# markrosoft/se-195-project-ray-tracer

Hardware: AMD Instinct MI355X
Metric: Mrays/sec + ms/frame @1920x1080 Cornell-64spp, 1/2/4/8 GPU; % HBM roofline (higher is better)
Workload: dtype f32; 1 GPU; smallpt Cornell 1920x1080 64spp RadiancePathTracing, one frame per step; spp=64, spheres=9, rows_per_gpu=1080, parallelism=single GPU

## Files before the change

se-195-project-ray-tracer_amd/csrc/smallpt.hip:

```cpp
#include "rt_common.h"
#include "rt_glibc_math.h"
#include "spt_policy.h"
#include "spt_layout.h"
#include "spt_accept.h"
#include "spt_rng.h"

namespace rt {
namespace smallpt {

using namespace sptlayout;
namespace acc = sptaccept;
constexpr float EPS = acc::EPS;
constexpr float PI_F = 3.14159265358979323846f;
constexpr int DIFF = 0, SPEC = 1;
#ifndef RT_SPT_QUNROLL
#define RT_SPT_QUNROLL 3
#endif

struct SphereGeo { float4 g; };

__device__ __forceinline__ float get_random_f(uint32_t &s0, uint32_t &s1)
{
    return __uint_as_float(sptrng::draw<true>(s0, s1));
}
// ... 55 lines not shown
    return id;
}

constexpr float DET_SAFE = 0x1p-96f;
template <class G, class F, class T>
__device__ __forceinline__ bool for_spheres_bf(const G &geo, const ray3 &r, F &&accept, T &&trip)
{
    const auto roots = [&](int i, float &t1, float &t2) {
        const float4 g = geo.at(i);
        const float opx = g.x - r.o.x, opy = g.y - r.o.y, opz = g.z - r.o.z;
        const float b = opx * r.d.x + opy * r.d.y + opz * r.d.z;
        const float det = b * b - (opx * opx + opy * opy + opz * opz) + g.w;
        const float sd = sqrt_nr(det);
        t1 = b - sd;
        t2 = b + sd;
        return fabsf(det);
    };
    bool bad = false;
    int i = geo.count() - 1;
#pragma unroll 1
    for (; i >= RT_SPT_QUNROLL - 1; i -= RT_SPT_QUNROLL) {
        float t1[RT_SPT_QUNROLL], t2[RT_SPT_QUNROLL];
        float m = roots(i, t1[0], t2[0]);
#pragma unroll
        for (int j = 1; j < RT_SPT_QUNROLL; j++) m = __builtin_fminf(m, roots(i - j, t1[j], t2[j]));
        trip(RT_SPT_QUNROLL);
#pragma unroll
        for (int j = 0; j < RT_SPT_QUNROLL; j++) accept(i - j, RT_SPT_QUNROLL - 1 - j, t1[j], t2[j]);
        bad = bad || m < DET_SAFE;
    }
#pragma unroll 1
    for (; i >= 0; i--) {
        float t1, t2;
        bad = bad || roots(i, t1, t2) < DET_SAFE;
        trip(1);
        accept(i, 0, t1, t2);
    }
    return bad;
}

template <bool COUNT, bool KEYED, class G>
__device__ __forceinline__ int query_bf(const G &geo, const ray3 &r, float &t, int &first)
{
    const float t_in = t;
    int id = -1;
    bool bad = false;
    if constexpr (KEYED && COUNT) {
        uint32_t tb = acc::limit_key(t_in);
        bad = for_spheres_bf(geo, r, [&](int i, int, float t1, float t2) {
            const bool take = acc::nearest_accept(tb, t1, t2);
            id = take ? i : id;
            first = (first < 0 && take) ? i : first;
        }, [](int) {});
        t = acc::nearest_result(tb, t_in);
    } else if constexpr (KEYED) {
        uint32_t tb = acc::limit_key(t_in);
        int since = -(1 << 30);
        bad = for_spheres_bf(geo, r, [&](int, int after, float t1, float t2) {
            since = acc::nearest_accept(tb, t1, t2) ? after : since;
        }, [&](int k) { since += k; });
        id = since;
        t = acc::nearest_result(tb, t_in);
    } else {
#pragma unroll RT_SPT_QUNROLL
        for (int i = geo.count() - 1; i >= 0; i--) {
            const float4 g = geo.at(i);
            const float opx = g.x - r.o.x, opy = g.y - r.o.y, opz = g.z - r.o.z;
            const float b = opx * r.d.x + opy * r.d.y + opz * r.d.z;
            const float det = b * b - (opx * opx + opy * opy + opz * opz) + g.w;
            bad = bad || fabsf(det) < DET_SAFE;
            const float sd = sqrt_nr(det);
            const float t1 = b - sd, t2 = b + sd;
            const float d = t1 > EPS ? t1 : t2;
            const bool take = d > EPS && d < t;
            t = take ? d : t;
            id = take ? i : id;
            if (COUNT) first = (first < 0 && take) ? i : first;
        }
    }
    if (wave_any(bad)) {
        t = t_in;
        first = -1;
        id = query<COUNT>(geo, r, t, first);
    }
    return id;
}

template <bool COUNT, class G>
__device__ __forceinline__ void query2_bf(const G &geo, const ray3 &r, float &t, int &id, const ray3 &rs, bool sh,
                                          float &ts, int &ids, int &firsts)
{
    const float t_in = t, ts_in = ts;
    int first = -1;
    id = -1;
    ids = -1;
    bool bad = false, occ = false;
#pragma unroll RT_SPT_QUNROLL
    for (int i = geo.count() - 1; i >= 0; i--) {
        const float4 g = geo.at(i);
        {
            const float opx = g.x - r.o.x, opy = g.y - r.o.y, opz = g.z - r.o.z;
            const float b = opx * r.d.x + opy * r.d.y + opz * r.d.z;
            const float det = b * b - (opx * opx + opy * opy + opz * opz) + g.w;
            bad = bad || fabsf(det) < 0x1p-96f;
            const float sd = sqrt_nr(det);
            const float t1 = b - sd, t2 = b + sd;
            const float d = t1 > EPS ? t1 : t2;
            const bool take = d > EPS && d < t;
            t = take ? d : t;
            id = take ? i : id;
        }
        {
            const float opx = g.x - rs.o.x, opy = g.y - rs.o.y, opz = g.z - rs.o.z;
            const float b = opx * rs.d.x + opy * rs.d.y + opz * rs.d.z;
            const float det = b * b - (opx * opx + opy * opy + opz * opz) + g.w;
            bad = bad || (sh && fabsf(det) < 0x1p-96f);
            const float sd = sqrt_nr(det);
            const float t1 = b - sd, t2 = b + sd;
            const float d = t1 > EPS ? t1 : t2;
            const bool take = d > EPS && d < ts;
            if (COUNT) {
                ts = take ? d : ts;
                ids = take ? i : ids;
                firsts = (firsts < 0 && take) ? i : firsts;
            } else {
                occ = occ || take;
            }
        }
    }
    if (!COUNT) ids = occ ? 0 : -1;
    if (wave_any(bad)) {
        t = t_in;
        id = query<COUNT>(geo, r, t, first);
        ts = ts_in;
        firsts = -1;
        ids = query<COUNT>(geo, rs, ts, firsts);
    }
}

template <class G>
__device__ __forceinline__ bool shadow_bf(const G &geo, const ray3 &rs, float maxt, bool have)
{
    uint32_t near = acc::KEY_NONE;
    const bool bad = for_spheres_bf(geo, rs, [&](int, int, float t1, float t2) { acc::any_accept(near, t1, t2); }, [](int) {});
    bool occ = acc::any_result(near, maxt);
    if (wave_any(have && bad)) {
        float ts = maxt;
        int first = -1;
        occ = query<false>(geo, rs, ts, first) >= 0;
    }
    return occ;
}

#include "spt_walk.h"

struct Counts { unsigned isect, isectp, samples; unsigned long long tests; };

#ifdef RT_SPT_PROF
enum { PB_ITER, PB_SHADOW, PB_NEAREST, PB_DIFF, PB_SPEC, PB_REFR, PB_LIGHT, PB_BOUNCE, PB_DONE,
       PB_WCALL, PB_WSTEP, PB_WLEAF, PB_WSHADE, PB_FLUSH,
       PB_FL_THRESH, PB_FL_SLOT, PB_FL_ENDS, PB_FL_EMIT, PB_FL_DRAIN, PB_N };
__device__ unsigned long long g_spt_prof[2 * PB_N];
#define SPT_PROF(b)                                                                        \
    do {                                                                                   \
        prof_l[b]++;                                                                       \
        if ((int)(threadIdx.x & 63) == __builtin_ctzll(__builtin_amdgcn_read_exec())) prof_w[b]++; \
    } while (0)
#else
#define SPT_PROF(b) do {} while (0)
#endif

#ifdef RT_SPT_TRACE
__device__ uint4 *g_spt_trace;
__device__ int g_spt_only_group = -1;
#endif

__device__ __forceinline__ int to_int(float x)
{
    const float c = (x < 0.f) ? 0.f : ((x > 1.f) ? 1.f : x);
    return rt::cvt_i32_x86(rtm::powf(c, 1.f / 2.2f) * 255.f + .5f);
}
__device__ __forceinline__ uint32_t pack_rgb(float r, float g, float b)
{
    return (uint32_t)to_int(r) | ((uint32_t)to_int(g) << 8) | ((uint32_t)to_int(b) << 16);
}

template <bool DL, bool COUNT, int GEO, bool DUAL = false, bool RAYS = false, int CG = 0>
__global__ void __launch_bounds__(1024, variant_of(GEO, DL, DUAL, COUNT, RAYS, CG).min_waves())
render_kernel(const rt_sphere *__restrict__ spheres, int nspheres, rt_camera cam,
              float *__restrict__ colors, const uint32_t *seeds_in,
              uint32_t *seeds_out, uint32_t *__restrict__ pixels, int w, int h,
              int row_begin, int row_end, int tiles_x, int ntiles, int nslots, int gstride, int first_sample,
              int nsamples, int prio_sched, const int *__restrict__ group_order, unsigned *__restrict__ group_cost,
              const float4 *__restrict__ g_geo, const float4 *__restrict__ g_emi,
              const float4 *__restrict__ g_col, const float4 *__restrict__ g_lrec, int nlights,
              BvhView bvh, unsigned long long *__restrict__ counters, int *__restrict__ work, int split,
              int nheavy, int sflags)
{
    constexpr Variant V = variant_of(GEO, DL, DUAL, COUNT, RAYS, CG);
    constexpr bool LDS = V.lds();
    constexpr bool PERSIST = V.persist();
    constexpr bool PARK = V.park();
    constexpr bool DQ = V.dq();
    constexpr int WAVE_DW = wave_dwords(DQ);
    constexpr int SQ_RING = RING_FIELD_DW;
    extern __shared__ __attribute__((aligned(16))) char smem[];
    const int park_off = park_offset(V, nspheres, nlights);
    constexpr bool HELD = V.held_addr();
    const auto park_ptr = [&]() {
        int t = (int)threadIdx.x;
        if constexpr (!HELD) asm volatile("" : "+v"(t));
        return (float *)(smem + park_off + PARK_HEAD_BYTES) + (t >> 6) * WAVE_DW + (t & 63);
    };
    const auto ring_ptr = [&]() {
        const int t = (int)threadIdx.x;
        return (float *)(smem + park_off + PARK_HEAD_BYTES) + (t >> 6) * WAVE_DW + RING_BASE_DW;
    };
    if (PARK && threadIdx.x == 0) {
        float4 *pc = (float4 *)(smem + park_off);
        pc[0] = make_float4(cam.x.x, cam.x.y, cam.x.z, 1.f / w);
        pc[1] = make_float4(cam.y.x, cam.y.y, cam.y.z, 1.f / h);
        pc[2] = make_float4(cam.dir.x, cam.dir.y, cam.dir.z, 0.f);
        pc[3] = make_float4(cam.orig.x, cam.orig.y, cam.orig.z, 0.f);
    }
    if (PARK && !LDS) __syncthreads();
    Scene S;
    if (LDS) {
        float4 *s = (float4 *)smem;
        const int nrec = scene_records(nspheres, nlights);
        for (int i = threadIdx.x; i < nrec; i += blockDim.x) s[i] = g_geo[i];
        __syncthreads();
        S.geo = s; S.emi = s + nspheres; S.col = s + 2 * nspheres; S.lrec = s + 3 * nspheres;
    } else {
        S.geo = g_geo; S.emi = g_emi; S.col = g_col; S.lrec = g_lrec;
    }
    S.nlights = nlights;
    S.n = nspheres;
    const DynGeo geo{S.geo, S.n};
    const uint4 *wL = (const uint4 *)smem;
    unsigned *wstk = nullptr;
    if (GEO == GEO_WIDE) {
        uint4 *d = (uint4 *)smem;
        for (int i = threadIdx.x; i < 7 * bvh.wnodes; i += blockDim.x) d[i] = bvh.wnode[i];
        if (COUNT)
            for (int i = threadIdx.x; i < 2 * bvh.wnodes; i += blockDim.x) d[7 * bvh.wnodes + i] = bvh.wmax[i];
        wstk = (unsigned *)(smem + wide_stack_offset(bvh.wnodes, COUNT)) +
               (size_t)(threadIdx.x >> 6) * WIDE_LEVEL_DW * (bvh.wdepth - 1);
        __syncthreads();
    }

    const int lane = threadIdx.x & 63, wave = threadIdx.x >> 6;
    constexpr bool SCHED = V.sched();
    constexpr bool CALLS = COUNT || RAYS;
    Counts cnt = {0, 0, 0, 0};
    SPT_PROF_ONLY(unsigned prof_l[PB_N] = {}, prof_w[PB_N] = {};)
    const int hs = PERSIST ? sptpolicy::split_hs(split) : 0;
    const int hw = sptpolicy::split_hw(split) ? sptpolicy::split_hw(split) : (4 << hs);
    const int nitems = 4 * nslots;
    const int n1 = PERSIST ? min(sptpolicy::nheavy_n1(nheavy), nitems) : 0;
    const int n2 = PERSIST ? min(sptpolicy::nheavy_n2(nheavy), nitems - n1) : 0;
    const int nwork = (n1 << hs) + (nitems - n1);
    const int nstatic = PERSIST ? min(min(hw, (int)(blockDim.x >> 6)) * (int)gridDim.x, n1 << hs) : 0;
    const auto fetch = [&]() {
        int v = 0;
        if (lane == __builtin_ctzll(__builtin_amdgcn_read_exec())) {
            v = -1;
            if (wave < hw && n1 > 0) {
                const int hv = atomicAdd(work + 2, 1) + nstatic;
                if (hv < (n1 << hs)) v = hv;
            }
            if (v < 0 && wave < 4 && n2 > 0) {
                const int hv = atomicAdd(work + 1, 1);
                if (hv < n2) v = (n1 << hs) + hv;
            }
            if (v < 0) v = (n1 << hs) + n2 + atomicAdd(work, 1);
        }
        return __builtin_amdgcn_readfirstlane(v);
    };
    int f = ((wave >> 2) * (int)gridDim.x + (int)blockIdx.x) * 4 + (wave & 3);
    if (PERSIST) {
        const int fs = wave * (int)gridDim.x + (int)blockIdx.x;
        f = (wave < hw && fs < (n1 << hs)) ? fs : __builtin_amdgcn_readfirstlane(fetch());
    }
    while (!PERSIST || f < nwork) {
    const bool heavy_ = f < (n1 << hs);
    const bool coop = GEO == GEO_WIDE && CG != 0 && heavy_;
    const int cg = coop ? CG : 0;
    const int item = heavy_ ? f >> hs : f - (n1 << hs) + n1;
    const int sub = heavy_ ? f & ((1 << hs) - 1) : 0;
    const int slot = item >> 2;
    const int grp = group_order ? (slot < nslots ? group_order[slot] : -1) : slot;
    const bool gvalid = (unsigned)grp < (unsigned)((ntiles + 3) >> 2);
    const int tile = grp * 4 + (item & 3);
    const int li = coop ? (sub << (6 - hs)) + (lane >> hs) : lane;
    const bool lead = !coop || (lane & (cg - 1)) == 0;
    unsigned long long t_start = 0;
    if (SCHED) t_start = __builtin_amdgcn_s_memrealtime();
    constexpr bool GSTORE = V.gstore();
#define GS_BASE() (smem + (size_t)((threadIdx.x >> 6) >> 2) * GS_BYTES)
    if (GSTORE) {
        if ((threadIdx.x & 255) == 0) *(int *)(GS_BASE() + GS_COUNT_OFF) = 0;
        __syncthreads();
    }
    int x = (tile % tiles_x) * 8 + (li & 7);
    int y = row_begin + (tile / tiles_x) * 8 * gstride + (li >> 3);
    const bool refill = COUNT && PERSIST && !heavy_;
    bool active = gvalid && tile < ntiles && x < w && y < row_end
                  SPT_TRACE(&& (g_spt_only_group < 0 || grp == g_spt_only_group));
    SPT_TRACE(unsigned tr_walk = 0, tr_leaf = 0, tr_trips = 0, tr_leafruns = 0, tr_queries = 0;
              const unsigned long long tr_c0 = __builtin_amdgcn_s_memtime();
              const unsigned long long tr_t0 = __builtin_amdgcn_s_memrealtime();
              unsigned tr_iters = 0;)
    if (active || refill || DQ) {
        int i = (h - y - 1) * w + x;
// ... 74 lines not shown
                        if (SCHED && group_cost) {
                            const unsigned dur = (unsigned)__builtin_amdgcn_s_memrealtime() - pix_t0;
                            if (sptpolicy::sflags_cost_max(sflags)) atomicMax(&group_cost[pgrp], dur);
                            else atomicAdd(&group_cost[pgrp], dur);
                        }
                    }
                    const unsigned long long need = __builtin_amdgcn_ballot_w64(want);
                    const int ncl = __builtin_popcountll(need);
                    const int rank = __builtin_amdgcn_mbcnt_hi((unsigned)(need >> 32),
                                                               __builtin_amdgcn_mbcnt_lo((unsigned)need, 0u));
                    const bool more = rf_p + ncl > 64;
                    const int f2 = more ? fetch() : nwork;
                    if (want) {
                        const int pos = rf_p + rank;
                        const int mf = pos < 64 ? rf_f : f2, mp = pos < 64 ? pos : pos - 64;
                        px_ok = false;
                        if (mf >= nwork) {
                            exhausted = true;
                        } else {
                            const int it = mf - (n1 << hs) + n1, sl = it >> 2;
                            const int g = group_order ? (sl < nslots ? group_order[sl] : -1) : sl;
                            const int tl = g * 4 + (it & 3);
                            x = (tl % tiles_x) * 8 + (mp & 7);
                            y = row_begin + (tl / tiles_x) * 8 * gstride + (mp >> 3);
                            if ((unsigned)g < (unsigned)((ntiles + 3) >> 2) && tl < ntiles && x < w && y < row_end) {
                                i = (h - y - 1) * w + x;
                                s0 = seeds_in[2 * (size_t)i];
                                s1 = seeds_in[2 * (size_t)i + 1];
                                col = mk(0.f, 0.f, 0.f);
                                if (first_sample > 0)
                                    col = mk(colors[3 * (size_t)i], colors[3 * (size_t)i + 1], colors[3 * (size_t)i + 2]);
                                k = 0;
                                need_cam = nsamples > 0;
                                px_ok = true;
                                pgrp = g;
                                pix_t0 = (unsigned)__builtin_amdgcn_s_memrealtime();
                            }
                        }
                    }
                    if (more) {
                        rf_f = f2;
                        rf_p += ncl - 64;
                    } else {
                        rf_p += ncl;
                    }
                }
            }
            if (need_bounce || need_cam) {
                SPT_PROF(PB_BOUNCE);
                const float f1 = get_random_f(s0, s1), f2 = get_random_f(s0, s1);
                const float x1 = __builtin_fmaf(f1, .5f, -1.f), x2 = __builtin_fmaf(f2, .5f, -1.f);
                const v3 wv = nl;
                const v3 a = (fabsf(wv.x) > .1f) ? mk(0.f, 1.f, 0.f) : mk(1.f, 0.f, 0.f);
                const v3 cu = vxcross(a, wv);
                float4 cmx = make_float4(cam.x.x, cam.x.y, cam.x.z, invW), cmy = make_float4(cam.y.x, cam.y.y, cam.y.z, invH);
                float4 cmd = make_float4(cam.dir.x, cam.dir.y, cam.dir.z, 0.f);
                float4 cmo = make_float4(cam.orig.x, cam.orig.y, cam.orig.z, 0.f);
                if constexpr (PARK) {
                    int o = park_off;
                    asm volatile("" : "+s"(o));
                    const float4 *pc = (const float4 *)(smem + o);
                    cmx = pc[0]; cmy = pc[1]; cmd = pc[2]; cmo = pc[3];
                }
                const float kcx = (x + __builtin_fmaf(f1, .5f, -1.5f)) * cmx.w - .5f;
                const float kcy = (y + __builtin_fmaf(f2, .5f, -1.5f)) * cmy.w - .5f;
                const v3 rdir = mk(cmx.x * kcx + cmy.x * kcy + cmd.x,
                                   cmx.y * kcx + cmy.y * kcy + cmd.y,
                                   cmx.z * kcx + cmy.z * kcy + cmd.z);
                const v3 vn = vnorm(need_bounce ? cu : rdir);
                if (need_bounce) {
                    const float r2s = sqrt_exact(x2);
                    const v3 v = vxcross(wv, vn);
                    float sn1, cs1, r2c;
                    if constexpr (V.draw_trig()) {
                        rtm::sincos_2pi_draw_bits(__float_as_uint(f1), x1, sn1, cs1);
                        r2c = sqrt_nr(1 - x2);
                    } else {
                        rtm::sincosf(2.f * PI_F * x1, sn1, cs1);
                        r2c = sqrt_exact(1 - x2);
                    }
                    const v3 u = vsmul(cs1 * r2s, vn);
                    v3 nd = vadd(u, vsmul(sn1 * r2s, v));
                    nd = vadd(nd, vsmul(r2c, wv));
                    ray.d = nd;
                } else {
                    v3 rorig = vsmul(0.1f, rdir);
                    rorig = vadd(rorig, mk(cmo.x, cmo.y, cmo.z));
                    ray.o = rorig;
                    ray.d = vn;
                }
                need_bounce = need_cam = false;
            }
            const bool live = !DQ || k < nsamples;
            bool drain = false;
            if constexpr (DQ) {
                drain = !wave_any(live);
                if (drain && q_count == 0) break;
            } else if (k >= nsamples) {
                if (!refill || exhausted) break;
                continue;
            }
            if (!refill && !wave_any(k < prio_next)) {
                prio_level++;
                prio_next = prio_level < 3 ? (nsamples * sptpolicy::prio_bound(prio_sched, prio_level)) >> 8 : nsamples;
                if (prio_level == 1) __builtin_amdgcn_s_setprio(2);
                else if (prio_level == 2) __builtin_amdgcn_s_setprio(1);
                else __builtin_amdgcn_s_setprio(0);
            }

            SPT_PROF(PB_ITER);
            SPT_TRACE(tr_iters++;)
            float t = (shadow && !DUAL) ? lmax : 1e20f;
            int first = -1;
            int id;
            bool done = false, lights = false, a_R = false;
            bool pushed = false;
            if constexpr (DQ) {
                id = -1;
                if (live) id = query_bf<COUNT, V.key_accept()>(geo, ray, t, first);
                bool f_emit = false, f_ends = false, f_diff = false;
                if (live && npend > 0) {
                    bool emit = false;
                    if (id >= 0) {
                        const float4 oe = S.emi[id];
                        emit = !((oe.x == 0.f) && (oe.x == 0.f) && (oe.z == 0.f));
                        f_diff = !emit && __float_as_int(oe.w) == DIFF;
                    }
                    f_emit = emit && specular;
                    f_ends = id < 0 || emit || depth >= 6;
                }
                while (true) {
                    const bool force = (f_emit && npend > npark) || (f_ends && npark > 0) || (f_diff && npend == 2);
                    if (q_count == 0 || !(sptpolicy::sq_flush(q_count, q_T) || drain || wave_any(force))) break;
                    const int m = sptpolicy::sq_pop(q_count);
                    const int e = sptpolicy::sq_wrap(q_head + lane);
                    const float *rg = ring_ptr();
                    ray3 rs;
                    rs.o = mk(rg[e], rg[SQ_RING + e], rg[2 * SQ_RING + e]);
                    rs.d = mk(rg[3 * SQ_RING + e], rg[4 * SQ_RING + e], rg[5 * SQ_RING + e]);
                    const float maxt = rg[6 * SQ_RING + e];
                    const bool have = lane < m;
                    SPT_PROF_ONLY(if (have) prof_l[PB_FLUSH]++; if (lane == 0) prof_w[PB_FLUSH]++;)
                    SPT_PROF_ONLY({
                        const int why = sptpolicy::sq_flush(q_count, q_T)        ? PB_FL_THRESH
                                        : wave_any(f_diff && npend == 2)         ? PB_FL_SLOT
                                        : wave_any(f_ends && npark > 0)          ? PB_FL_ENDS
                                        : wave_any(f_emit && npend > npark)      ? PB_FL_EMIT
                                                                                 : PB_FL_DRAIN;
                        _Pragma("unroll") for (int b = PB_FL_THRESH; b <= PB_FL_DRAIN; b++) {
                            if (have && b == why) prof_l[b]++;
                            if (lane == 0 && b == why) prof_w[b]++;
                        }
                    })
                    const bool occ = shadow_bf(geo, rs, maxt, have);
                    const unsigned long long unocc = __builtin_amdgcn_ballot_w64(have && !occ);
                    while (npend > 0) {
                        const int rel = sptpolicy::sq_rel(pidx & 255, q_head);
                        if (rel >= m) break;
                        const bool lit = (unocc >> rel) & 1ull;
                        if (npark > 0) {
                            float *p = park_ptr();
                            if (lit) {
                                p[64 * SLOT_RAD] = p[64 * SLOT_RAD] + pc0.x;
                                p[64 * (SLOT_RAD + 1)] = p[64 * (SLOT_RAD + 1)] + pc0.y;
                                p[64 * (SLOT_RAD + 2)] = p[64 * (SLOT_RAD + 2)] + pc0.z;
                            }
                            npark--;
                            if (npark == 0)
                                fold(mk(p[64 * SLOT_RAD], p[64 * (SLOT_RAD + 1)], p[64 * (SLOT_RAD + 2)]),
                                     first_sample + k - 1);
                        } else if (lit) {
                            rad = vadd(rad, pc0);
                        }
                        npend--;
                        pidx >>= 8;
                        if (npend > 0) {
                            const float *p = park_ptr();
                            pc0 = mk(p[64 * SLOT_PEND], p[64 * (SLOT_PEND + 1)], p[64 * (SLOT_PEND + 2)]);
                        }
                    }
                    q_head = __builtin_amdgcn_readfirstlane(sptpolicy::sq_wrap(q_head + m));
                    q_count = __builtin_amdgcn_readfirstlane(q_count - m);
                }
            } else if constexpr (DUAL) {
                if (wave_any(shadow)) {
                    float ts = lmax;
                    int ids, firsts = -1;
                    ray3 rs;
                    rs.o = hit;
                    rs.d = sdir;
                    query2_bf<COUNT>(geo, ray, t, id, rs, shadow, ts, ids, firsts);
                    if (shadow) {
                        SPT_PROF(PB_SHADOW);
                        cnt.isectp++;
                        cnt.tests += firsts >= 0 ? (unsigned)(S.n - firsts) : (unsigned)S.n;
                        if (ids < 0) {
                            const float4 le = S.lrec[2];
                            const v3 ld = vsmul(lw, mk(le.x, le.y, le.z));
                            rad = vadd(rad, vmul(thr, ld));
                        }
                        shadow = false;
                        done = fin;
                    }
                } else {
                    id = query_bf<COUNT, V.key_accept()>(geo, ray, t, first);
                }
            } else if constexpr (GEO == GEO_BVH) {
                SPT_TRACE(const unsigned long long tr_w0 = __builtin_amdgcn_s_memtime(); tr_queries += !walking;)
                if (!walking) bvh_begin<COUNT>(bvh, ray, shadow, t, walk);
                walking = !bvh_walk<COUNT>(bvh, ray, shadow, walk);
                SPT_TRACE(tr_walk += (unsigned)(__builtin_amdgcn_s_memtime() - tr_w0);)
                if (walking) continue;
                t = walk.t;
                id = walk.id;
                first = id;
            } else if constexpr (GEO == GEO_WIDE) {
                SPT_TRACE(const unsigned long long tr_w0 = __builtin_amdgcn_s_memtime(); tr_queries += !walking;)
                if (!walking) wide_begin<COUNT>(bvh, ray, shadow, t, walk);
                if constexpr (CG != 0)
                    walking = coop ? !wide_walk_coop<COUNT, (CG ? CG : 8)>(bvh, wL, wstk, ray, shadow, walk, split)
                                   : !wide_walk<COUNT>(bvh, wL, wstk, ray, shadow, walk, split);
                else
                    walking = !wide_walk<COUNT>(bvh, wL, wstk, ray, shadow, walk, split);
                SPT_TRACE(tr_walk += (unsigned)(__builtin_amdgcn_s_memtime() - tr_w0);)
                if (walking) continue;
                SPT_PROF(PB_WSHADE);
                t = walk.t;
                id = walk.id;
                first = id;
            } else {
                id = query_bf<COUNT, V.key_accept()>(geo, ray, t, first);
            }
            float dp = 0.f, inv_sign = 1.f;
            if (DQ && !live) {
            } else if (DUAL && fin) {
            } else if (shadow && !DUAL) {
                SPT_PROF(PB_SHADOW);
                cnt.isectp++;
                cnt.tests += first >= 0 ? (unsigned)(S.n - first) : (unsigned)S.n;
                if (id < 0) {
                    const float4 le = S.lrec[3 * li + 2];
                    lsum = vadd(lsum, vsmul(lw, mk(le.x, le.y, le.z)));
                }
                li++;
                lights = true;
                shadow = false;
            } else {
                cnt.isect++;
                cnt.tests += S.n;
                if (id < 0) {
                    done = true;
                } else {
                    SPT_PROF(PB_NEAREST);
                    const float4 og = S.geo[id], oe = S.emi[id], oc = S.col[id];
                    hit = vadd(ray.o, vsmul(t, ray.d));
                    v3 normal = vsub(hit, mk(og.x, og.y, og.z));
                    normal = vnorm(normal);
                    dp = vdot(normal, ray.d);
                    inv_sign = -1.f * (dp > 0 ? 1.f : -1.f);
                    nl = vsmul(inv_sign, normal);
                    const int refl = __float_as_int(oe.w);
                    if (!((oe.x == 0.f) && (oe.x == 0.f) && (oe.z == 0.f))) {
                        if (specular) {
                            v3 e = vsmul(fabsf(dp), mk(oe.x, oe.y, oe.z));
                            e = vmul(thr, e);
                            rad = vadd(rad, e);
                        }
                        done = true;
                    } else if (refl == DIFF) {
                        SPT_PROF(PB_DIFF);
                        specular = false;
                        thr = vmul(thr, mk(oc.x, oc.y, oc.z));
                        lsum = mk(0.f, 0.f, 0.f);
                        li = 0;
                        lights = true;
                    } else if (refl == SPEC) {
                        SPT_PROF(PB_SPEC);
                        specular = true;
                        v3 nd = vsmul(2.f * vdot(normal, ray.d), normal);
                        nd = vsub(ray.d, nd);
                        thr = vmul(thr, mk(oc.x, oc.y, oc.z));
                        ray.d = nd;
                    } else {
                        SPT_PROF(PB_REFR);
                        specular = true;
                        a_R = true;
                    }
                    depth++;
                    done = done || (!lights && !a_R && depth > 6);
                }
            }

            bool a_L = lights && li < S.nlights;
            bool lights_done = lights && !a_L;
            const bool was_R = a_R;
            const auto pass_a = [&](const bool with_r) {
                {
                    SPT_PROF(PB_LIGHT);
                    const int lj = li < S.nlights ? li : 0;
                    const float4 lg = S.lrec[3 * lj];
                    const float4 lc = S.lrec[3 * lj + 1];
                    const v3 normal = vsmul(inv_sign, nl);
                    const bool into = dp <= 0.f;
                    const float nnt = into ? nc / nt : nt / nc;
                    const float ddn = inv_sign * dp;
                    const float cos2t = 1.f - nnt * nnt * (1.f - ddn * ddn);
                    const bool tir = cos2t < 0.f;
                    float g1 = 2.f, x2 = 0.f;
                    if (a_L || (with_r && !tir)) g1 = get_random_f(s0, s1);
                    const float x1 = __builtin_fmaf(g1, .5f, -1.f);
                    if (a_L) x2 = get_random(s0, s1);
                    const float zz = 1.f - 2.f * x2;
                    const float q = 1.f - zz * zz;
                    const float sq = sqrt_exact((!with_r || a_L) ? ((0.f > q) ? 0.f : q) : (tir ? 1.f : cos2t));
                    float sp_sin, sp_cos;
                    if constexpr (V.draw_trig()) rtm::sincos_2pi_draw_bits(__float_as_uint(g1), x1, sp_sin, sp_cos);
                    else rtm::sincosf(2.f * PI_F * x1, sp_sin, sp_cos);
                    const v3 unit = mk(sq * sp_cos, sq * sp_sin, zz);
                    v3 sp = vsmul(lc.w, unit);
                    sp = vadd(sp, mk(lg.x, lg.y, lg.z));
                    const v3 vl = vsub(sp, hit);
                    const float kk = (into ? 1.f : -1.f) * (ddn * nnt + sq);
                    const v3 vr = vsub(vsmul(nnt, ray.d), vsmul(kk, normal));
                    const v3 vv = (!with_r || a_L) ? vl : vr;
                    const float dd = vdot(vv, vv);
                    float len, ilen;
                    if (!wave_any(!sqrt_nr_ok(dd))) {
                        len = sqrt_nr(dd);
                        ilen = rcp_nr(len);
                    } else {
                        len = sqrt_rn(dd);
                        ilen = 1.f / len;
                    }
                    const v3 vn = vsmul(ilen, vv);
                    const float dv = vdot(vn, (!with_r || a_L) ? unit : normal);
                    const float wo = -dv;
                    const float wi = vdot(vn, nl);
                    const bool lit = a_L && !(dv > 0.f) && wi > 0.f;
                    const float a = nt - nc, b = nt + nc;
                    const float R0 = a * a / (b * b);
                    const float c = 1 - (into ? -ddn : dv);
                    const float Re = R0 + (1 - R0) * c * c * c * c * c;
                    const float Tr = 1.f - Re;
                    const float P = .25f + .5f * Re;
                    const bool refl_pick = x1 < P;
                    const bool l_lane = !with_r || a_L;
                    const float num = l_lane ? (4.f * PI_F * lc.w * lc.w) * wi * wo : (refl_pick ? Re : Tr);
                    const float den = l_lane ? len * len : (refl_pick ? P : 1.f - P);
                    const float quo = num / den;
                    unsigned long long pm = 0;
                    if constexpr (DQ) pm = __builtin_amdgcn_ballot_w64(lit);
                    if (!with_r || a_L) {
                        if (DQ && lit) {
                            const int rank = __builtin_amdgcn_mbcnt_hi((unsigned)(pm >> 32),
                                                                       __builtin_amdgcn_mbcnt_lo((unsigned)pm, 0u));
                            const int pos = sptpolicy::sq_push_pos(q_head, q_count, rank);
                            float *rg = ring_ptr();
                            rg[pos] = hit.x;
                            rg[SQ_RING + pos] = hit.y;
                            rg[2 * SQ_RING + pos] = hit.z;
                            rg[3 * SQ_RING + pos] = vn.x;
                            rg[4 * SQ_RING + pos] = vn.y;
                            rg[5 * SQ_RING + pos] = vn.z;
                            rg[6 * SQ_RING + pos] = len - EPS;
                            const float4 le = S.lrec[2];
                            const v3 c = vmul(thr, vsmul(quo, mk(le.x, le.y, le.z)));
                            if (npend == 0) {
                                pc0 = c;
                                pidx = pos;
                            } else {
                                float *p = park_ptr();
                                p[64 * SLOT_PEND] = c.x;
                                p[64 * (SLOT_PEND + 1)] = c.y;
                                p[64 * (SLOT_PEND + 2)] = c.z;
                                pidx |= pos << 8;
                            }
                            npend++;
                            pushed = true;
                            a_L = false;
                            lights_done = true;
                        } else if (lit) {
                            if (DUAL) {
                                sdir = vn;
                            } else {
                                ray.d = vn;
                            }
                            lmax = len - EPS;
                            lw = quo;
                            shadow = true;
                            a_L = false;
                            if (DUAL) lights_done = true;
                        } else {
                            li++;
                            a_L = li < S.nlights;
                            lights_done = !a_L;
                        }
                    } else {
                        const float4 oc = S.col[id];
                        v3 nd = vsmul(2.f * dp, normal);
                        nd = vsub(ray.d, nd);
                        if (tir) {
                            thr = vmul(thr, mk(oc.x, oc.y, oc.z));
                            ray.d = nd;
                        } else {
                            thr = vsmul(quo, thr);
                            thr = vmul(thr, mk(oc.x, oc.y, oc.z));
                            ray.d = refl_pick ? nd : vn;
                        }
                        a_R = false;
                    }
                }
            };
            if ((GEO == GEO_BVH || GEO == GEO_WIDE) && sptpolicy::sflags_no_refr(sflags)) {
                if (a_L) pass_a(false);
            } else if (a_L || a_R) {
                pass_a(true);
            }
            if (S.nlights > 1) {
                while (wave_any(a_L)) {
                    if (a_L) pass_a(false);
                }
            }
            if constexpr (DQ)
                q_count = __builtin_amdgcn_readfirstlane(
                    q_count + __builtin_popcountll(__builtin_amdgcn_ballot_w64(pushed)));
            if (was_R) done = depth > 6;
            if (lights_done) {
                if (!DUAL) rad = vadd(rad, vmul(thr, lsum));
                if (DL) {
                    done = true;
                } else if (depth > 6) {
                    (void)get_random(s0, s1);
                    (void)get_random(s0, s1);
                    if (DUAL && shadow) fin = true;
                    else done = true;
                } else {
                    need_bounce = true;
                }
            }
            if (done) {
                SPT_PROF(PB_DONE);
                const int current = first_sample + k;
                if constexpr (DQ) {
                    if (npend > 0) {
                        float *p = park_ptr();
                        p[64 * SLOT_RAD] = rad.x;
                        p[64 * (SLOT_RAD + 1)] = rad.y;
                        p[64 * (SLOT_RAD + 2)] = rad.z;
                        npark = npend;
                    } else {
                        fold(rad, current);
                    }
                } else if constexpr (PARK) {
                    fold(rad, current);
                } else if (current == 0) {
                    col = rad;
                } else {
                    const float k1 = (float)current;
                    const float k2 = rcp_nr(k1 + 1.f);
                    col.x = (col.x * k1 + rad.x) * k2;
                    col.y = (col.y * k1 + rad.y) * k2;
                    col.z = (col.z * k1 + rad.z) * k2;
                }
                cnt.samples++;
                if (CALLS && (cnt.isect | cnt.isectp) >= 0x80000000u) {
                    atomicAdd(counters, (unsigned long long)cnt.isect);
                    atomicAdd(counters + 1, (unsigned long long)cnt.isectp);
                    cnt.isect = cnt.isectp = 0;
                }
                k++;
                need_cam = k < nsamples;
                fin = false;
                rad = mk(0.f, 0.f, 0.f);
                thr = mk(1.f, 1.f, 1.f);
                depth = 0;
                specular = true;
            }
        }
        if (GSTORE) {
            float *gs_col = (float *)GS_BASE();
            uint32_t *gs_seed = (uint32_t *)(GS_BASE() + GS_SEED_OFF), *gs_px = (uint32_t *)(GS_BASE() + GS_PX_OFF);
            const int c = (wave & 3) * 8 + (lane & 7), r = lane >> 3;
            if (nsamples > 0) {
                gs_col[r * 96 + 3 * c] = col.x;
                gs_col[r * 96 + 3 * c + 1] = col.y;
                gs_col[r * 96 + 3 * c + 2] = col.z;
                gs_px[r * 32 + c] = pack_rgb(col.x, col.y, col.z);
            }
            gs_seed[r * 64 + 2 * c] = s0;
            gs_seed[r * 64 + 2 * c + 1] = s1;
        } else if (lead && !refill && (!DQ || active)) {
            if (PARK && nsamples > 0) {
                const float *p = park_ptr();
                col = mk(p[64 * SLOT_COL], p[64 * (SLOT_COL + 1)], p[64 * (SLOT_COL + 2)]);
            }
            if (nsamples > 0) {
                colors[3 * (size_t)i] = col.x;
                colors[3 * (size_t)i + 1] = col.y;
                colors[3 * (size_t)i + 2] = col.z;
                pixels[(size_t)y * w + x] = pack_rgb(col.x, col.y, col.z);
            }
            seeds_out[2 * (size_t)i] = s0;
            seeds_out[2 * (size_t)i + 1] = s1;
        }
        SPT_PROF_ONLY(for (int b = 0; b < 3; b++) {
            prof_l[PB_WCALL + b] += walk.pf_l[b];
            prof_w[PB_WCALL + b] += walk.pf_w[b];
        })
        SPT_TRACE(if (GEO == GEO_BVH || GEO == GEO_WIDE) {
            tr_leaf = walk.tr_leaf;
            tr_trips = walk.tr_trips;
            tr_leafruns = walk.tr_leafruns;
        })
    }
    if (GSTORE) {
        const float *gs_col = (const float *)GS_BASE();
        const uint32_t *gs_seed = (const uint32_t *)(GS_BASE() + GS_SEED_OFF);
        const uint32_t *gs_px = (const uint32_t *)(GS_BASE() + GS_PX_OFF);
        __builtin_amdgcn_fence(__ATOMIC_RELEASE, "workgroup");
        int old = 0;
        if (lane == 0) old = atomicAdd((int *)(GS_BASE() + GS_COUNT_OFF), 1);
        old = __shfl(old, 0, 64);
        if (old == 3) {
            __builtin_amdgcn_fence(__ATOMIC_ACQUIRE, "workgroup");
            const auto pix = [&](int r, int c, int &xx, int &yy) {
                const int tl = grp * 4 + (c >> 3);
                xx = (tl % tiles_x) * 8 + (c & 7);
                yy = row_begin + (tl / tiles_x) * 8 * gstride + r;
                return gvalid && tl < ntiles && xx < w && yy < row_end;
            };
            int xx, yy;
            if (nsamples > 0) {
#pragma unroll 4
                for (int k = 0; k < 12; k++) {
                    const int j = k * 64 + lane, r = j / 96, c3 = j % 96, c = c3 / 3;
                    if (pix(r, c, xx, yy)) colors[3 * ((size_t)(h - yy - 1) * w + xx) + (c3 - 3 * c)] = gs_col[j];
                }
#pragma unroll
                for (int k = 0; k < 4; k++) {
                    const int j = k * 64 + lane, r = j >> 5, c = j & 31;
                    if (pix(r, c, xx, yy)) pixels[(size_t)yy * w + xx] = gs_px[j];
                }
            }
#pragma unroll
            for (int k = 0; k < 8; k++) {
                const int j = k * 64 + lane, r = j >> 6, c2 = j & 63, c = c2 >> 1;
                if (pix(r, c, xx, yy)) seeds_out[2 * ((size_t)(h - yy - 1) * w + xx) + (c2 & 1)] = gs_seed[j];
            }
        }
    }
#undef GS_BASE
    if (SCHED && group_cost && gvalid && lane == 0 && !refill) {
        const unsigned dur = (unsigned)(__builtin_amdgcn_s_memrealtime() - t_start);
        if (sptpolicy::sflags_cost_max(sflags)) atomicMax(&group_cost[grp], dur);
        else atomicAdd(&group_cost[grp], dur);
    }
    SPT_TRACE({
        const unsigned long long t1 = __builtin_amdgcn_s_memrealtime();
        unsigned mx = tr_iters;
        _Pragma("unroll")
        for (int off = 32; off > 0; off >>= 1) mx = max(mx, (unsigned)__shfl_xor((int)mx, off, 64));
        const unsigned sum = (unsigned)wave_sum_u64(tr_iters);
        const size_t wv = (size_t)f;
        const unsigned tr_tot = (unsigned)(__builtin_amdgcn_s_memtime() - tr_c0);
        unsigned ph[6] = {tr_walk, tr_leaf, tr_trips, tr_leafruns, tr_queries, tr_tot};
        _Pragma("unroll")
        for (int q = 0; q < 6; q++)
            _Pragma("unroll")
            for (int off = 32; off > 0; off >>= 1) ph[q] = max(ph[q], (unsigned)__shfl_xor((int)ph[q], off, 64));
        if (lane == 0 && g_spt_trace) {
            g_spt_trace[4 * wv] = make_uint4((unsigned)tr_t0, (unsigned)t1, __builtin_amdgcn_s_getreg(0xF804),
                                             __builtin_amdgcn_s_getreg(0xF814));
            g_spt_trace[4 * wv + 1] = make_uint4(sum, mx, (unsigned)grp, ph[5]);
            g_spt_trace[4 * wv + 2] = make_uint4(ph[0], ph[1], ph[2], ph[3]);
            g_spt_trace[4 * wv + 3] = make_uint4(ph[4], 0u, 0u, 0u);
        }
    })
    if (CALLS && PERSIST && sptpolicy::split_coop(split)) {
        if (!lead) cnt = Counts{0, 0, 0, 0};
// ... 1061 lines not shown
```

se-195-project-ray-tracer_amd/csrc/spt_policy.h:

```cpp
#ifndef SPT_POLICY_H
#define SPT_POLICY_H

#include <stdio.h>
#include <stdlib.h>
#include <algorithm>
#include <string>

#ifdef __HIPCC__
#define SPT_HD __host__ __device__ __forceinline__
#else
#define SPT_HD
#endif

namespace sptpolicy {

inline int pack_split(int hs, bool coop, int hw, int budget, int batch, int stop)
{
    return (int)((unsigned)hs | (coop ? 4u : 0u) | ((unsigned)hw << 3) | ((unsigned)budget << 8) |
                 ((unsigned)batch << 16) | ((unsigned)stop << 24));
}
SPT_HD constexpr int split_hs(int split) { return split & 3; }
SPT_HD constexpr bool split_coop(int split) { return split & 4; }
SPT_HD constexpr int split_hw(int split) { return (split >> 3) & 31; }
SPT_HD constexpr int split_budget(int split) { return (split >> 8) & 255; }
SPT_HD constexpr int split_batch(int split) { return (split >> 16) & 255; }
SPT_HD constexpr int split_stop(int split) { return (split >> 24) & 255; }

inline int pack_nheavy(int n1, int n2)
{
    return (int)((unsigned)std::min(n1, 0xffff) | ((unsigned)std::min(n2, 0xffff) << 16));
}
SPT_HD constexpr int nheavy_n1(int nheavy) { return nheavy & 0xffff; }
SPT_HD constexpr int nheavy_n2(int nheavy) { return (nheavy >> 16) & 0xffff; }

inline int pack_sflags(bool no_refr, bool cost_max, int sq = 0)
{
    return (no_refr ? 1 : 0) | (cost_max ? 4 : 0) | ((sq & 127) << 8);
}
SPT_HD constexpr bool sflags_no_refr(int sflags) { return sflags & 1; }
SPT_HD constexpr bool sflags_cost_max(int sflags) { return sflags & 4; }
SPT_HD constexpr int sflags_sq(int sflags) { return (sflags >> 8) & 127; }

constexpr int SQ_RING = 112;
constexpr int SQ_DEFAULT = 49;
SPT_HD constexpr int sq_capacity(int T) { return T + 63; }
SPT_HD constexpr int sq_max_threshold() { return SQ_RING - 63; }
SPT_HD constexpr int sq_threshold(int T) { return T < 1 ? SQ_DEFAULT : (T > sq_max_threshold() ? sq_max_threshold() : T); }
SPT_HD constexpr int sq_wrap(int i) { return i >= SQ_RING ? i - SQ_RING : i; }
SPT_HD constexpr bool sq_flush(int count, int T) { return count >= T; }
SPT_HD constexpr int sq_pop(int count) { return count < 64 ? count : 64; }
SPT_HD constexpr int sq_push_pos(int head, int count, int rank) { return sq_wrap(sq_wrap(head + count) + rank); }
SPT_HD constexpr int sq_rel(int pos, int head) { return pos - head < 0 ? pos - head + SQ_RING : pos - head; }

inline int pack_prio(int a, int b, int c) { return (a & 255) | ((b & 255) << 8) | ((c & 255) << 16); }
SPT_HD constexpr int prio_bound(int prio_sched, int level) { return (prio_sched >> (8 * level)) & 255; }

struct SptTune {
    int coop = -1, coop_g = 0, coop_waves = -1, routed = -1;
    int budget = 16, batch = 16, stop = -1;
    int prio[3] = {-1, -1, -1};
    int wpb = 0, blocks = 0;
    int sq = 0;
};
inline SptTune spt_tune_parse(const char *e)
{
    SptTune t;
    if (!e) return t;
    std::string all(e);
    size_t pos = 0;
    while (pos < all.size()) {
        size_t end = all.find(',', pos);
        if (end == std::string::npos) end = all.size();
        const std::string kv = all.substr(pos, end - pos);
        pos = end + 1;
        const size_t eq = kv.find('=');
        if (eq == std::string::npos) continue;
        const std::string k = kv.substr(0, eq);
        const char *v = kv.c_str() + eq + 1;
        if (k == "coop") t.coop = std::max(atoi(v), 0);
        else if (k == "coop_g") t.coop_g = atoi(v) == 4 ? 4 : (atoi(v) == 2 ? 2 : 8);
        else if (k == "coop_waves") t.coop_waves = std::min(std::max(atoi(v), 0), 16);
        else if (k == "routed") t.routed = std::max(atoi(v), 0);
        else if (k == "walk") sscanf(v, "%d/%d/%d", &t.budget, &t.batch, &t.stop);
        else if (k == "prio") sscanf(v, "%d/%d/%d", &t.prio[0], &t.prio[1], &t.prio[2]);
        else if (k == "wpb") t.wpb = atoi(v) == 16 ? 16 : 4;
        else if (k == "blocks") t.blocks = std::max(atoi(v), 0);
        else if (k == "sq") t.sq = std::min(std::max(atoi(v), 1), 64);
    }
    return t;
}
inline SptTune spt_tune() { return spt_tune_parse(getenv("RT_SPT_TUNE")); }

constexpr int WIDE_WPB = 16;

struct Shape {
    int tiles_x, ntiles, gstride, wpb, nblocks;
    int work = 0;
    int nslots = 0;
    bool wide = false;
    const int *order = nullptr;
    unsigned *cost = nullptr;
    bool tiers = true;
    bool cost_max = false;
    SptTune tune;
};
inline Shape launch_shape(int cus, bool wide, int w, int r0, int r1, int gstride, int nlist, const SptTune &tune)
{
    Shape g;
    g.tune = tune;
    g.wide = wide;
    g.tiles_x = (w + 7) / 8;
    g.gstride = gstride;
    const int groups = (r1 - r0 + 7) / 8;
    g.ntiles = g.tiles_x * ((groups + gstride - 1) / gstride);
    const int work = nlist > 0 ? 4 * nlist : g.ntiles;
    g.work = work;
    const double wps = (double)work / (4.0 * cus);
    g.wpb = (wps <= 4.0 || (wps > 6.0 && wps <= 8.0)) ? 16 : 4;
    if (g.tune.wpb) g.wpb = g.tune.wpb;
    g.nblocks = (work + g.wpb - 1) / g.wpb;
    g.nslots = nlist > 0 ? nlist : g.nblocks * (g.wpb / 4);
    if (wide) {
        g.wpb = WIDE_WPB;
        g.nblocks = std::min(cus, (work + g.wpb - 1) / g.wpb);
        if (g.tune.blocks) g.nblocks = g.tune.blocks;
        g.nslots = nlist > 0 ? nlist : (g.ntiles + 3) / 4;
    }
    return g;
}

inline int prio_schedule(const Shape &g)
{
    int a = 64, b = 128, c = 192;
    if (g.wpb == 16) { a = 128; b = 192; c = 224; }
    if (g.tune.prio[0] >= 0) { a = g.tune.prio[0]; b = g.tune.prio[1]; c = g.tune.prio[2]; }
    return pack_prio(a, b, c);
}

struct Tiers { int n1 = 0, n2 = 0, cg = 0, hw = 0, stop = 32; };
inline Tiers heavy_tiers(const Shape &g, int cus)
{
    const SptTune &tu = g.tune;
    Tiers t;
    int n1 = 0, n2 = 0;
    if (g.wide && g.order && g.tiers) {
        n2 = std::min(4 * g.nblocks, 4 * g.nslots);
        const double wps = (double)g.work / (4.0 * cus);
        int hw = 0, cg = 8;
        if (wps <= 5.0) {
            n1 = 2 * cus;
            hw = 16;
        } else if (wps <= 10.0) {
            n1 = 4 * cus;
            hw = 16;
            cg = 4;
        } else if (wps <= 20.0) {
            n1 = 4 * cus;
            cg = 2;
        }
        if (tu.coop_g) cg = tu.coop_g;
        if (tu.coop >= 0) n1 = tu.coop;
        if (tu.coop_waves >= 0) hw = tu.coop_waves;
        if (n1 > 0) n2 = 0;
        if (tu.routed >= 0) n2 = tu.routed;
        n1 = std::min(n1, 4 * g.nslots);
        n2 = std::min(n2, 4 * g.nslots - n1);
        t.cg = n1 > 0 ? cg : 0;
        t.hw = n1 > 0 ? hw : 0;
    }
    t.n1 = n1;
    t.n2 = n2;
    t.stop = tu.stop >= 0 ? tu.stop : (n1 > 0 ? 16 : 32);
    return t;
}

inline int split_word(const Shape &g, const Tiers &t)
{
    const int hs = t.cg == 8 ? 3 : t.cg == 4 ? 2 : t.cg == 2 ? 1 : 0;
    return pack_split(hs, t.cg != 0, t.hw, std::min(std::max(g.tune.budget, 1), 255),
                      std::min(std::max(g.tune.batch, 0), 64), std::min(std::max(t.stop, 0), 64));
}

}

#endif
```

Baseline: 88450 Mrays/s.

## Resolve shadow-queue owners branchlessly and specialize DUAL path for single light

Replaces the per-lane while loop that retires pending shadow results one by one with a closed-form owner resolution that handles up to two pending entries at once, and returns the unoccluded mask directly from a new ballot-based shadow helper. Pending contributions are now always written to the park slot with selects instead of branching. The DUAL path is specialized to assume a single light, removing the multi-light loop and the light-index bookkeeping. The aim is less divergence and fewer loop iterations in the flush path, at the cost of extra LDS writes and an implicit single-light assumption in DUAL mode.

After: 91080 Mrays/s (median of 6 runs). 3.0% higher.

```diff
diff --git a/se-195-project-ray-tracer_amd/csrc/smallpt.hip b/se-195-project-ray-tracer_amd/csrc/smallpt.hip
--- a/se-195-project-ray-tracer_amd/csrc/smallpt.hip
+++ b/se-195-project-ray-tracer_amd/csrc/smallpt.hip
@@ -231,6 +231,23 @@
     return occ;
 }
 
+template <class G>
+__device__ __forceinline__ unsigned long long shadow_bf_unocc(const G &geo, const ray3 &rs, float maxt, bool have)
+{
+    uint32_t near = acc::KEY_NONE;
+    const bool bad = for_spheres_bf(geo, rs, [&](int, int, float t1, float t2) { acc::any_accept(near, t1, t2); }, [](int) {});
+    const unsigned long long hm = __builtin_amdgcn_ballot_w64(have);
+    uint32_t lim = acc::limit_key(maxt);
+    asm volatile("" : "+v"(lim));
+    unsigned long long un = hm & ~__builtin_amdgcn_ballot_w64(near < lim);
+    if (wave_any(have && bad)) {
+        float ts = maxt;
+        int first = -1;
+        un = hm & __builtin_amdgcn_ballot_w64(query<false>(geo, rs, ts, first) < 0);
+    }
+    return un;
+}
+
 #include "spt_walk.h"
 
 struct Counts { unsigned isect, isectp, samples; unsigned long long tests; };
@@ -238,7 +255,8 @@
 #ifdef RT_SPT_PROF
 enum { PB_ITER, PB_SHADOW, PB_NEAREST, PB_DIFF, PB_SPEC, PB_REFR, PB_LIGHT, PB_BOUNCE, PB_DONE,
        PB_WCALL, PB_WSTEP, PB_WLEAF, PB_WSHADE, PB_FLUSH,
-       PB_FL_THRESH, PB_FL_SLOT, PB_FL_ENDS, PB_FL_EMIT, PB_FL_DRAIN, PB_N };
+       PB_FL_THRESH, PB_FL_SLOT, PB_FL_ENDS, PB_FL_EMIT, PB_FL_DRAIN,
+       PB_OW_ROUND, PB_OW_FOLD, PB_OW_ONE, PB_OW_TWO, PB_N };
 __device__ unsigned long long g_spt_prof[2 * PB_N];
 #define SPT_PROF(b)                                                                        \
     do {                                                                                   \
@@ -619,32 +637,41 @@
                             if (lane == 0 && b == why) prof_w[b]++;
                         }
                     })
-                    const bool occ = shadow_bf(geo, rs, maxt, have);
-                    const unsigned long long unocc = __builtin_amdgcn_ballot_w64(have && !occ);
-                    while (npend > 0) {
-                        const int rel = sptpolicy::sq_rel(pidx & 255, q_head);
-                        if (rel >= m) break;
-                        const bool lit = (unocc >> rel) & 1ull;
-                        if (npark > 0) {
-                            float *p = park_ptr();
-                            if (lit) {
-                                p[64 * SLOT_RAD] = p[64 * SLOT_RAD] + pc0.x;
-                                p[64 * (SLOT_RAD + 1)] = p[64 * (SLOT_RAD + 1)] + pc0.y;
-                                p[64 * (SLOT_RAD + 2)] = p[64 * (SLOT_RAD + 2)] + pc0.z;
+                    const unsigned long long unocc = shadow_bf_unocc(geo, rs, maxt, have);
+                    const sptpolicy::SqOwners ow = sptpolicy::sq_owners(pidx, npend, q_head, m, unocc);
+                    if (ow.r0) {
+                        SPT_PROF(PB_OW_ROUND);
+                        SPT_PROF_ONLY(if (ow.r1) prof_l[PB_OW_ROUND]++;)
+                        SPT_PROF_ONLY(if (ow.r1) SPT_PROF(PB_OW_TWO); else SPT_PROF(PB_OW_ONE);)
+                        const int nres = sptpolicy::sq_owners_resolved(ow);
+                        const int nparked = sptpolicy::sq_owners_parked(nres, npark);
+                        float *p = park_ptr();
+                        v3 pc1 = pc0;
+                        if (npend == 2) pc1 = mk(p[64 * SLOT_PEND], p[64 * (SLOT_PEND + 1)], p[64 * (SLOT_PEND + 2)]);
+                        if (nparked > 0) {
+                            v3 pr = mk(p[64 * SLOT_RAD], p[64 * (SLOT_RAD + 1)], p[64 * (SLOT_RAD + 2)]);
+                            const bool add0 = ow.lit0, add1 = nparked == 2 && ow.lit1;
+                            if (add0) pr = vadd(pr, pc0);
+                            if (add1) pr = vadd(pr, pc1);
+                            if (add0 || add1) {
+                                p[64 * SLOT_RAD] = pr.x;
+                                p[64 * (SLOT_RAD + 1)] = pr.y;
+                                p[64 * (SLOT_RAD + 2)] = pr.z;
                             }
-                            npark--;
-                            if (npark == 0)
-                                fold(mk(p[64 * SLOT_RAD], p[64 * (SLOT_RAD + 1)], p[64 * (SLOT_RAD + 2)]),
-                                     first_sample + k - 1);
-                        } else if (lit) {
+                            if (nparked == npark) {
+                                SPT_PROF(PB_OW_FOLD);
+                                int prev = first_sample + k - 1;
+                                asm volatile("" : "+v"(prev));
+                                fold(pr, prev);
+                            }
+                        } else if (ow.lit0) {
                             rad = vadd(rad, pc0);
                         }
-                        npend--;
-                        pidx >>= 8;
-                        if (npend > 0) {
-                            const float *p = park_ptr();
-                            pc0 = mk(p[64 * SLOT_PEND], p[64 * (SLOT_PEND + 1)], p[64 * (SLOT_PEND + 2)]);
-                        }
+                        if (ow.lit1 && nparked < 2) rad = vadd(rad, pc1);
+                        npark -= nparked;
+                        npend -= nres;
+                        pidx = sptpolicy::sq_owners_shift(pidx, nres);
+                        pc0 = pc1;
                     }
                     q_head = __builtin_amdgcn_readfirstlane(sptpolicy::sq_wrap(q_head + m));
                     q_count = __builtin_amdgcn_readfirstlane(q_count - m);
@@ -739,7 +766,7 @@
                         specular = false;
                         thr = vmul(thr, mk(oc.x, oc.y, oc.z));
                         lsum = mk(0.f, 0.f, 0.f);
-                        li = 0;
+                        if constexpr (!DUAL) li = 0;
                         lights = true;
                     } else if (refl == SPEC) {
                         SPT_PROF(PB_SPEC);
@@ -754,17 +781,17 @@
                         a_R = true;
                     }
                     depth++;
-                    done = done || (!lights && !a_R && depth > 6);
+                    done = done || (!lights && (DUAL || !a_R) && depth > 6);
                 }
             }
 
-            bool a_L = lights && li < S.nlights;
+            bool a_L = DUAL ? lights : lights && li < S.nlights;
             bool lights_done = lights && !a_L;
             const bool was_R = a_R;
             const auto pass_a = [&](const bool with_r) {
                 {
                     SPT_PROF(PB_LIGHT);
-                    const int lj = li < S.nlights ? li : 0;
+                    const int lj = DUAL ? 0 : (li < S.nlights ? li : 0);
                     const float4 lg = S.lrec[3 * lj];
                     const float4 lc = S.lrec[3 * lj + 1];
                     const v3 normal = vsmul(inv_sign, nl);
@@ -792,7 +819,8 @@
                     const v3 vv = (!with_r || a_L) ? vl : vr;
                     const float dd = vdot(vv, vv);
                     float len, ilen;
-                    if (!wave_any(!sqrt_nr_ok(dd))) {
+                    const bool in_range = !wave_any(!sqrt_nr_ok(dd));
+                    if (DUAL ? __builtin_expect(in_range, 1) : in_range) {
                         len = sqrt_nr(dd);
                         ilen = rcp_nr(len);
                     } else {
@@ -832,16 +860,13 @@
                             rg[6 * SQ_RING + pos] = len - EPS;
                             const float4 le = S.lrec[2];
                             const v3 c = vmul(thr, vsmul(quo, mk(le.x, le.y, le.z)));
-                            if (npend == 0) {
-                                pc0 = c;
-                                pidx = pos;
-                            } else {
-                                float *p = park_ptr();
-                                p[64 * SLOT_PEND] = c.x;
-                                p[64 * (SLOT_PEND + 1)] = c.y;
-                                p[64 * (SLOT_PEND + 2)] = c.z;
-                                pidx |= pos << 8;
-                            }
+                            const bool first_term = npend == 0;
+                            float *p = park_ptr();
+                            p[64 * SLOT_PEND] = c.x;
+                            p[64 * (SLOT_PEND + 1)] = c.y;
+                            p[64 * (SLOT_PEND + 2)] = c.z;
+                            pc0 = mk(first_term ? c.x : pc0.x, first_term ? c.y : pc0.y, first_term ? c.z : pc0.z);
+                            pidx = first_term ? pos : (pidx | pos << 8);
                             npend++;
                             pushed = true;
                             a_L = false;
@@ -857,6 +882,9 @@
                             shadow = true;
                             a_L = false;
                             if (DUAL) lights_done = true;
+                        } else if constexpr (DUAL) {
+                            a_L = false;
+                            lights_done = true;
                         } else {
                             li++;
                             a_L = li < S.nlights;
@@ -883,15 +911,19 @@
             } else if (a_L || a_R) {
                 pass_a(true);
             }
-            if (S.nlights > 1) {
-                while (wave_any(a_L)) {
-                    if (a_L) pass_a(false);
+            if constexpr (!DUAL) {
+                if (S.nlights > 1) {
+                    while (wave_any(a_L)) {
+                        if (a_L) pass_a(false);
+                    }
                 }
             }
             if constexpr (DQ)
                 q_count = __builtin_amdgcn_readfirstlane(
                     q_count + __builtin_popcountll(__builtin_amdgcn_ballot_w64(pushed)));
-            if (was_R) done = depth > 6;
+            if constexpr (!DUAL) {
+                if (was_R) done = depth > 6;
+            }
             if (lights_done) {
                 if (!DUAL) rad = vadd(rad, vmul(thr, lsum));
                 if (DL) {
diff --git a/se-195-project-ray-tracer_amd/csrc/spt_policy.h b/se-195-project-ray-tracer_amd/csrc/spt_policy.h
--- a/se-195-project-ray-tracer_amd/csrc/spt_policy.h
+++ b/se-195-project-ray-tracer_amd/csrc/spt_policy.h
@@ -51,6 +51,20 @@
 SPT_HD constexpr int sq_pop(int count) { return count < 64 ? count : 64; }
 SPT_HD constexpr int sq_push_pos(int head, int count, int rank) { return sq_wrap(sq_wrap(head + count) + rank); }
 SPT_HD constexpr int sq_rel(int pos, int head) { return pos - head < 0 ? pos - head + SQ_RING : pos - head; }
+
+struct SqOwners {
+    bool r0, r1;
+    bool lit0, lit1;
+};
+SPT_HD constexpr SqOwners sq_owners(int pidx, int npend, int head, int m, unsigned long long unocc)
+{
+    const int rel0 = sq_rel(pidx & 255, head), rel1 = sq_rel((pidx >> 8) & 255, head);
+    const bool r0 = npend > 0 && rel0 < m, r1 = r0 && npend > 1 && rel1 < m;
+    return SqOwners{r0, r1, r0 && ((unocc >> (rel0 & 63)) & 1ull) != 0, r1 && ((unocc >> (rel1 & 63)) & 1ull) != 0};
+}
+SPT_HD constexpr int sq_owners_resolved(const SqOwners &o) { return o.r1 ? 2 : (o.r0 ? 1 : 0); }
+SPT_HD constexpr int sq_owners_parked(int n, int npark) { return n < npark ? n : npark; }
+SPT_HD constexpr int sq_owners_shift(int pidx, int n) { return pidx >> (8 * n); }
 
 inline int pack_prio(int a, int b, int c) { return (a & 255) | ((b & 255) << 8) | ((c & 255) << 16); }
 SPT_HD constexpr int prio_bound(int prio_sched, int level) { return (prio_sched >> (8 * level)) & 255; }
```
